# scroll-tech/scroll-prover

Hardware: AMD Instinct MI355X
Metric: BN254 MSM G1-adds/sec at k=26 (higher is better)
Workload: dtype u32 (9x29-bit limbs of 254-bit Montgomery integers; v_mad_u64_u32); 1 GPU; BN254 G1 Pippenger MSM, 2^26 uniform random scalars x synthetic SRS points, inputs resident in HBM; point-range shards over 1 GPU(s), RCCL all-gather of 96-B partials; log_n=26, window_bits=22, windows=12, parallelism=point-range x1, one rank per GPU, srs_window_tables=True

## Files before the change

### scroll-prover_amd/csrc/lib_msm.hip

```cpp
#define ZK_FRSCAN_DEVICE_ONLY 1
#include "msm.hpp"
#define ZK_G2_DEVICE_ONLY 1
#include "msm_g2.hpp"
#include "msm_seg.hpp"
#include "lib_common.hpp"

namespace mi355 {
using mi355zk::Fixup; using mi355zk::PassPlan; using mi355zk::PlanIn; using mi355zk::TableShape;

static_assert(sizeof(fe_t) == 32 && sizeof(g1_affine_t) == 64 && sizeof(g1_jac_t) == 96, "ABI element sizes");
static_assert(sizeof(g1_xyzz_t) == 128 && sizeof(g1_xyzz29_t) == 144, "device record sizes (workspace layout, 16-byte vector accesses)");
static_assert(sizeof(g1_xyzz29_t) == mi355zk::GROUP_G1.rec_bytes && sizeof(g2_xyzz_t) == mi355zk::GROUP_G2.rec_bytes, "the planner's record sizes");

int msm_tu_init_device() {
  HIPCHK(hipFuncSetAttribute((const void *)k_sort_l1_scatter_split<24>, hipFuncAttributeMaxDynamicSharedMemorySize, 160 * 1024));
  HIPCHK(hipFuncSetAttribute((const void *)k_sort_l1_scatter_split<16>, hipFuncAttributeMaxDynamicSharedMemorySize, 160 * 1024));
  HIPCHK(hipFuncSetAttribute((const void *)k_sort_l1_scatter_split<8>, hipFuncAttributeMaxDynamicSharedMemorySize, 160 * 1024));
  HIPCHK(hipFuncSetAttribute((const void *)k_sort_l2_scatter_split<16>, hipFuncAttributeMaxDynamicSharedMemorySize, 160 * 1024));
  HIPCHK(hipFuncSetAttribute((const void *)k_sort_l2_scatter_split<8>, hipFuncAttributeMaxDynamicSharedMemorySize, 160 * 1024));
  return MI355_OK;
}

static PlanIn plan_in() {
  PlanIn in; in.k = static_cast<const mi355zk::Knobs &>(g); in.auto_max_c = g_proc.msm_auto_max_c; in.chunk_min_log = g.msm_chunk_min_log;
// ... 2 lines not shown
}

struct PreTable { const g1_affine_t *table = nullptr; uint64_t row_stride = 0; int c = 0, w = 0; };
static TableShape tab_of(const PreTable *pre) { return pre && pre->table ? TableShape{pre->c, pre->w} : TableShape{}; }
const PreTable *pre_advance(const PreTable *pre, uint64_t lo, PreTable &store) {
  if (!pre) return nullptr;
  store = *pre; if (store.table) store.table += lo;
  return &store;
}

struct Roles {
  const char *prefix; std::string sfx;
  template <class T> int get(const char *name, size_t bytes, T *&ptr) const { return ws_get((std::string(prefix) + name + sfx).c_str(), bytes, (void **)&ptr); }
};

struct MsmStreams { hipStream_t a, b, c; };
struct SpanNames { const char *total, *digits, *sort, *l1, *hist, *l2, *accumulate, *fixup, *tail; };

template <class H> struct PassArgs {
  const typename H::base_t *bases; uint64_t row_stride;
  PolyPtrs inl; const fe_t *const *polys_dev;
  typename H::Ops::out_t *out;
  MsmSlot *slot; MsmStreams st;
  uint32_t set_index = 0, set_count = 1;
  bool skip_tail = false;
  bool normalise = true;
};

struct G1Pass {
  using Ops = G1Ops; using base_t = g1_affine_t;
  static constexpr mi355zk::MsmGroup GROUP = mi355zk::GROUP_G1;
  static constexpr bool FOLD = true, G1_SCHEDULES = true;
  static constexpr SpanNames SPAN{"msm_total", "msm_digits", "msm_sort", "sort_l1", "sort_hist", "sort_l2", "msm_accumulate", "msm_reduce", nullptr};
  static constexpr const char *TRACE = "msm_g1", *N_LIMIT = "msm: n must be < 2^31"; static constexpr double TRACE_BYTES = 96.0;
  static void accumulate(const PassPlan &pl, const PassArgs<G1Pass> &a, const uint32_t *sorted, const uint32_t *offsets, g1_xyzz29_t *buckets, g1_xyzz29_t *part, int32_t *part_id, hipStream_t s) {
    hipLaunchKernelGGL(k_msm_accumulate, dim3(pl.blocks), dim3(256), 0, s, a.bases, sorted, offsets, (uint32_t)pl.nbuckets, buckets, part, part_id, pl.seg_arg, log2_ceil(pl.n), a.row_stride);
  }
};
struct G2Pass {
  using Ops = G2Ops; using base_t = g2_affine_t;
  static constexpr mi355zk::MsmGroup GROUP = mi355zk::GROUP_G2;
  static constexpr bool FOLD = false, G1_SCHEDULES = false;
  static constexpr SpanNames SPAN{"msm_g2_total", "msm_g2_digits", "msm_g2_sort", "g2_sort_l1", "g2_sort_hist", "g2_sort_l2", "msm_g2_accumulate", "msm_g2_fixup", "msm_g2_reduce"};
  static constexpr const char *TRACE = "msm_g2", *N_LIMIT = "msm_g2: n must be < 2^31"; static constexpr double TRACE_BYTES = 160.0;
  static void accumulate(const PassPlan &pl, const PassArgs<G2Pass> &a, const uint32_t *sorted, const uint32_t *offsets, g2_xyzz_t *buckets, g2_xyzz_t *part, int32_t *part_id, hipStream_t s) {
    hipLaunchKernelGGL(k_msm_g2_accumulate, dim3(pl.blocks), dim3(256), 0, s, a.bases, sorted, offsets, (uint32_t)pl.nbuckets, buckets, part, part_id, pl.seg_arg);
  }
};

static void g1_bases(PassArgs<G1Pass> &a, const PassPlan &pl, const g1_affine_t *bases, const PreTable *pre) {
  if (pl.shared) { a.bases = pre->table; a.row_stride = pre->row_stride; } else { a.bases = bases; a.row_stride = 0; }
}

int msm_stage_polys(const fe_t *const *polys_host, uint32_t M, const Roles &ws, hipStream_t s, PolyPtrs &inl, const fe_t **&polys_dev) {
  if (M <= 8) { for (uint32_t m = 0; m < M; m++) inl.p[m] = polys_host[m]; return MI355_OK; }
  CHK(ws.get("polys", (size_t)M * sizeof(void *), polys_dev));
  g.polys_stage.assign(polys_host, polys_host + M);
  HIPCHK(hipMemcpyAsync(polys_dev, g.polys_stage.data(), (size_t)M * sizeof(void *), hipMemcpyHostToDevice, s));
  HIPCHK(hipStreamSynchronize(s));
  return MI355_OK;
}

template <class G, class F> void with_lanes(bool quad, F &&launch) {
  if constexpr (G::QUAD) { if (quad) { launch(std::integral_constant<int, 4>{}); return; } }
  launch(std::integral_constant<int, 1>{});
}

template <class H> int msm_sort_stage(const PassPlan &pl, const MsmPlan &P, const PolyPtrs &inl, const fe_t *const *polys_dev, uint32_t *offsets, uint32_t *sorted, hipStream_t s) {
  const uint64_t emax = pl.emax;
  const uint32_t nbuckets = (uint32_t)pl.nbuckets, M = pl.M;
  SortPlan S; S.n = P.n; S.windows = M * P.windows; S.wpp = P.windows; S.nb = P.nb;
  S.fb = pl.fb; S.cb_bits = pl.cb_bits;
  S.shared = pl.shared ? 1 : 0; S.nshift = log2_ceil(pl.n);
  S.regions = pl.regions; S.t1 = pl.t1; S.t2 = pl.t2;
  const uint32_t tiles1 = pl.tiles1, l2_tiles_max = pl.l2_tiles_max;
  const uint32_t vwindows = M * P.windows;

  uint32_t *enc, *hist, *cursor, *scan_sums, *coarse_hist, *coarse_off, *coarse_cursor, *tile_start;
  CHK(ws_get("msm.digits", emax * 4, (void **)&enc));
  uint32_t *pairs_lo = nullptr; uint16_t *pairs_hi = nullptr;
  CHK(ws_get("msm.pairs_lo", emax * 4 + 64, (void **)&pairs_lo)); CHK(ws_get("msm.pairs_hi", emax * 2 + 64, (void **)&pairs_hi));
  CHK(ws_get("msm.hist", ((size_t)nbuckets + 1) * 4, (void **)&hist));
  CHK(ws_get("msm.cursor", ((size_t)nbuckets + 1) * 4, (void **)&cursor));
  CHK(ws_get("msm.coarse_hist", ((size_t)S.regions + 1) * 4, (void **)&coarse_hist));
  CHK(ws_get("msm.coarse_off", ((size_t)S.regions + 1) * 4, (void **)&coarse_off));
  CHK(ws_get("msm.coarse_cursor", ((size_t)S.regions + 1) * 4, (void **)&coarse_cursor));
  CHK(ws_get("msm.tile_start", ((size_t)S.regions + 1) * 4, (void **)&tile_start));
  const uint32_t scan_n = nbuckets + 1, scan_blocks = ceil_div(scan_n, SCAN_BLOCK * SCAN_ITEMS);
  const uint32_t cscan_n = S.regions + 1, cscan_blocks = ceil_div(cscan_n, SCAN_BLOCK * SCAN_ITEMS);
  CHK(ws_get("msm.scan_sums", (size_t)(scan_blocks + cscan_blocks) * 4, (void **)&scan_sums));
  const int grid_stream = g.prop.multiProcessorCount * 8;
  {
    Scope sc(H::SPAN.digits, s);
    HIPCHK(hipMemsetAsync(coarse_hist, 0, ((size_t)S.regions + 1) * 4, s));
    const dim3 dgrid(grid_stream / M > 0 ? grid_stream / M : 1, M);
    hipLaunchKernelGGL(k_msm_digits<H::FOLD>, dgrid, dim3(256), (size_t)S.regions * 4, s, inl, polys_dev, enc, P, coarse_hist, S.fb, S.cb_bits, S.shared);
  }
  {
    Scope sc(H::SPAN.sort, s);
    HIPCHK(hipMemsetAsync(hist, 0, ((size_t)nbuckets + 1) * 4, s));
    hipLaunchKernelGGL(k_scan_partial, dim3(cscan_blocks), dim3(SCAN_BLOCK), 0, s, coarse_hist, scan_sums + scan_blocks, cscan_n);
    hipLaunchKernelGGL(k_scan_block_sums, dim3(1), dim3(SCAN_BLOCK), 0, s, scan_sums + scan_blocks, cscan_blocks);
    hipLaunchKernelGGL(k_scan_final, dim3(cscan_blocks), dim3(SCAN_BLOCK), 0, s, coarse_hist, scan_sums + scan_blocks, coarse_off, coarse_cursor, cscan_n);
    {
      Scope s1(H::SPAN.l1, s);
      const uint32_t CBp = ((1u << S.cb_bits) + 1) & ~1u;
      const size_t lds1 = (size_t)(3 * CBp + 32 + SORT_SPLIT_TMAX) * 4 + (size_t)S.t1 * 6;
      if (S.t1 == 24576) hipLaunchKernelGGL(k_sort_l1_scatter_split<24>, dim3(tiles1 * vwindows), dim3(1024), lds1, s, enc, coarse_cursor, pairs_lo, pairs_hi, S);
      else if (S.t1 == 16384) hipLaunchKernelGGL(k_sort_l1_scatter_split<16>, dim3(tiles1 * vwindows), dim3(1024), lds1, s, enc, coarse_cursor, pairs_lo, pairs_hi, S);
      else hipLaunchKernelGGL(k_sort_l1_scatter_split<8>, dim3(tiles1 * vwindows), dim3(1024), lds1, s, enc, coarse_cursor, pairs_lo, pairs_hi, S);
    }
    hipLaunchKernelGGL(k_sort_tile_prefix, dim3(1), dim3(SCAN_BLOCK), 0, s, coarse_off, tile_start, S);
    { Scope s2(H::SPAN.hist, s);
    hipLaunchKernelGGL(k_sort_l2_hist_split, dim3(l2_tiles_max), dim3(256), 0, s, (const uint16_t *)pairs_hi, coarse_off, tile_start, hist, S); }
    hipLaunchKernelGGL(k_scan_partial, dim3(scan_blocks), dim3(SCAN_BLOCK), 0, s, hist, scan_sums, scan_n);
    hipLaunchKernelGGL(k_scan_block_sums, dim3(1), dim3(SCAN_BLOCK), 0, s, scan_sums, scan_blocks);
    hipLaunchKernelGGL(k_scan_final, dim3(scan_blocks), dim3(SCAN_BLOCK), 0, s, hist, scan_sums, offsets, cursor, scan_n);
    {
      Scope s3(H::SPAN.l2, s);
      const size_t lds2 = (size_t)(3 * (1u << S.fb) + 32) * 4 + (size_t)S.t2 * 6;
      if (S.t2 == 8192) hipLaunchKernelGGL(k_sort_l2_scatter_split<8>, dim3(l2_tiles_max), dim3(1024), lds2, s, (const uint32_t *)pairs_lo, (const uint16_t *)pairs_hi, coarse_off, tile_start, cursor, sorted, S);
      else hipLaunchKernelGGL(k_sort_l2_scatter_split<16>, dim3(l2_tiles_max), dim3(1024), lds2, s, (const uint32_t *)pairs_lo, (const uint16_t *)pairs_hi, coarse_off, tile_start, cursor, sorted, S);
    }
  }
  return MI355_OK;
}

template <class G> int msm_segfix_levels(const int32_t *part_id, const typename G::rec_t *part, uint32_t tn, typename G::rec_t *buckets, hipStream_t s, const Roles &ws) {
  using rec_t = typename G::rec_t;
  uint32_t N = 2 * tn; const uint32_t waves1 = ceil_div(N, 64);
  const size_t cap = (size_t)2 * waves1 + (size_t)waves1 / 8 + 512;
  int32_t *lv_ids; rec_t *lv_recs;
  CHK(ws.get("segfix_ids", cap * 4, lv_ids)); CHK(ws.get("segfix_recs", cap * sizeof(rec_t), lv_recs));
  const int32_t *cur_ids = part_id; const rec_t *cur_recs = part; size_t used = 0;
  while (N > 64) {
    const uint32_t waves = ceil_div(N, 64);
    hipLaunchKernelGGL(k_msm_segfix<G>, dim3(ceil_div(N, 256)), dim3(256), 0, s, cur_ids, cur_recs, N, buckets, lv_ids + used, lv_recs + used, 0);
    cur_ids = lv_ids + used; cur_recs = lv_recs + used; used += (size_t)2 * waves; N = 2 * waves;
  }
  hipLaunchKernelGGL(k_msm_segfix<G>, dim3(1), dim3(64), 0, s, cur_ids, cur_recs, N, buckets, (int32_t *)nullptr, (rec_t *)nullptr, 1);
  return MI355_OK;
}

struct FixupLists {
  uint32_t *big_list, *big_count, *huge_list, *huge_count; g1_xyzz29_t *huge_part;
  int get(const PassPlan &pl, const Roles &ws) {
    CHK(ws.get("big_list", ((size_t)pl.big_cap * 3 + 1) * 4, big_list)); big_count = big_list + (size_t)pl.big_cap * 3;
    CHK(ws.get("huge_list", ((size_t)pl.huge_cap * 3 + 1) * 4, huge_list)); huge_count = huge_list + (size_t)pl.huge_cap * 3;
    return ws.get("huge_part", (size_t)pl.huge_cap * FIXUP_SLICES * sizeof(g1_xyzz29_t), huge_part);
  }
};
static void msm_fixup_per_bucket(const PassPlan &pl, const FixupLists &fl, const uint32_t *offsets, g1_xyzz29_t *buckets, g1_xyzz29_t *part, int32_t *part_id, hipStream_t s) {
  const uint32_t nbuckets = (uint32_t)pl.nbuckets;
  auto fixup = [&](auto kernel, uint64_t threads) {
    hipLaunchKernelGGL(kernel, dim3(ceil_div(threads, 256)), dim3(256), 0, s, offsets, nbuckets, buckets, part, part_id, pl.seg_arg, pl.tn, fl.big_list, fl.big_count, pl.big_cap, fl.huge_list, fl.huge_count, pl.huge_cap, pl.serial_max, pl.huge_min);
  };
  if (pl.fixup == Fixup::Quad) fixup(k_msm_fixup<4, 4>, (uint64_t)nbuckets * 16);
  else if (pl.fixup == Fixup::FourLanes) fixup(k_msm_fixup<4, 1>, (uint64_t)nbuckets * 4);
  else fixup(k_msm_fixup<1, 1>, nbuckets);
  hipLaunchKernelGGL(k_msm_fixup_big, dim3(pl.big_cap), dim3(256), 0, s, buckets, part, part_id, fl.big_list, fl.big_count);
  hipLaunchKernelGGL(k_msm_fixup_huge, dim3(pl.huge_cap * FIXUP_SLICES), dim3(256), 0, s, part, part_id, fl.huge_list, fl.huge_count, fl.huge_part, pl.huge_cap);
  hipLaunchKernelGGL(k_msm_fixup_huge_fold, dim3(pl.huge_cap), dim3(64), 0, s, buckets, fl.huge_list, fl.huge_count, (const g1_xyzz29_t *)fl.huge_part);
}

template <class G> int msm_reduce_tail(const PassPlan &pl, const typename G::rec_t *buckets, typename G::out_t *out_dev, bool normalise, hipStream_t s, const Roles &ws) {
  using rec_t = typename G::rec_t;
  const uint32_t nb = 1u << (pl.c - 1), wpp = pl.wpp(), sets = pl.sets(), chunks_per_set = pl.chunks_per_set, nchunks = chunks_per_set * sets;
  rec_t *chunk_out, *tree_a, *tree_b, *window_sums;
  CHK(ws.get("chunk_out", (size_t)nchunks * sizeof(rec_t), chunk_out));
  { const size_t lvl = (size_t)ceil_div(chunks_per_set, 64 * TREE_PER_THREAD) * sets + 1;
    CHK(ws.get("tree_a", lvl * sizeof(rec_t), tree_a)); CHK(ws.get("tree_b", lvl * sizeof(rec_t), tree_b)); }
  CHK(ws.get("window_sums", (size_t)sets * sizeof(rec_t), window_sums));
  with_lanes<G>(pl.quad_sums, [&](auto q) {
    constexpr int Q = decltype(q)::value;
    hipLaunchKernelGGL((k_msm_bucket_reduce<G, Q>), dim3(ceil_div((uint64_t)nchunks * Q, 128)), dim3(128), 0, s, buckets, chunk_out, nb, sets, pl.chunk);
  });
  const rec_t *cur = chunk_out; uint32_t cnt = chunks_per_set; rec_t *bufs[2] = {tree_a, tree_b}; int which = 0;
  while (true) {
    const bool coop = G::QUAD && pl.tree_quad(cnt);
    const uint32_t outn = ceil_div(cnt, (coop ? 64u : 256u) * TREE_PER_THREAD);
    rec_t *dst = outn == 1 ? window_sums : bufs[which];
    with_lanes<G>(coop, [&](auto q) { hipLaunchKernelGGL((k_msm_tree_sum<G, decltype(q)::value>), dim3(outn, sets), dim3(256), 0, s, cur, cnt, dst, outn); });
    if (outn == 1) break;
    cur = dst; cnt = outn; which ^= 1;
  }
  with_lanes<G>(pl.quad_final, [&](auto q) {
    hipLaunchKernelGGL((k_msm_final<G, decltype(q)::value>), dim3(pl.M), dim3(64), 0, s, (const rec_t *)window_sums, wpp, pl.shared ? 0u : pl.c, out_dev, normalise ? 1 : 0);
  });
  HIPCHK(hipGetLastError());
  return MI355_OK;
}

template <class H> int msm_pass(const PassPlan &pl, const PassArgs<H> &a) {
// ... 721 lines not shown
```

### scroll-prover_amd/csrc/msm.hpp

```cpp
#pragma once
#include "fp_asm.hpp"
#include "g1_29.hpp"
#include "frscan.hpp"
#include "msm_plan.hpp"

namespace zk {

#if defined(__HIPCC__)

struct MsmPlan {
  uint32_t n;
  uint32_t c;
  uint32_t windows;
  uint32_t nb;
  uint32_t seg;
  uint32_t batch;
};

__device__ __forceinline__ g1_affine_t load_affine(const g1_affine_t *p) {
  g1_affine_t r; r.x = g_load(&p->x); r.y = g_load(&p->y); return r;
}
__device__ __forceinline__ g1_affine_t load_affine_nt(const g1_affine_t *p) {
  const uint32_t *q = reinterpret_cast<const uint32_t *>(p); g1_affine_t r;
#pragma unroll
  for (int i = 0; i < 8; i++) { r.x.l[i] = __builtin_nontemporal_load(q + i); r.y.l[i] = __builtin_nontemporal_load(q + 8 + i); }
  return r;
}
__device__ __forceinline__ g1_xyzz_t load_xyzz(const g1_xyzz_t *p) {
  g1_xyzz_t r; r.x = g_load(&p->x); r.y = g_load(&p->y); r.zz = g_load(&p->zz); r.zzz = g_load(&p->zzz); return r;
}
__device__ __forceinline__ void store_xyzz(g1_xyzz_t *p, const g1_xyzz_t &v) {
  g_store(&p->x, v.x); g_store(&p->y, v.y); g_store(&p->zz, v.zz); g_store(&p->zzz, v.zzz);
}

__device__ __forceinline__ void store_xyzz29(g1_xyzz29_t *p, const g1_xyzz29_t &v) {
  const uint32_t *w = reinterpret_cast<const uint32_t *>(&v); uint4 *q = reinterpret_cast<uint4 *>(p);
#pragma unroll
  for (int i = 0; i < 9; i++) q[i] = make_uint4(w[4 * i], w[4 * i + 1], w[4 * i + 2], w[4 * i + 3]);
}
__device__ __forceinline__ g1_xyzz29_t load_xyzz29(const g1_xyzz29_t *p) {
  g1_xyzz29_t v; uint32_t *w = reinterpret_cast<uint32_t *>(&v); const uint4 *q = reinterpret_cast<const uint4 *>(p);
#pragma unroll
  for (int i = 0; i < 9; i++) { const uint4 a = q[i]; w[4 * i] = a.x; w[4 * i + 1] = a.y; w[4 * i + 2] = a.z; w[4 * i + 3] = a.w; }
  return v;
}

__device__ __forceinline__ g1_xyzz29_t shfl_down_xyzz29(const g1_xyzz29_t &v, uint32_t o) {
  g1_xyzz29_t r; const uint32_t *s = reinterpret_cast<const uint32_t *>(&v); uint32_t *d = reinterpret_cast<uint32_t *>(&r);
#pragma unroll
  for (int i = 0; i < 36; i++) d[i] = __shfl_down(s[i], o);
  return r;
}
__device__ __forceinline__ g1_xyzz29_t shfl_xor_xyzz29(const g1_xyzz29_t &v, uint32_t o) {
  g1_xyzz29_t r; const uint32_t *s = reinterpret_cast<const uint32_t *>(&v); uint32_t *d = reinterpret_cast<uint32_t *>(&r);
#pragma unroll
  for (int i = 0; i < 36; i++) d[i] = __shfl_xor(s[i], o);
  return r;
}

template <int J> __device__ __forceinline__ fe29_t quad_bcast(const fe29_t &v) {
  fe29_t r;
#pragma unroll
  for (int i = 0; i < 9; i++) {
    int x = __builtin_amdgcn_mov_dpp((int)v.l[i], J * 0x55, 0xf, 0xf, true);
    asm volatile("" : "+v"(x));
    r.l[i] = (uint32_t)x;
  }
  return r;
}
__device__ __forceinline__ fe29_t quad_sel(uint32_t q, const fe29_t a0, const fe29_t a1, const fe29_t a2, const fe29_t a3) {
  fe29_t r;
#pragma unroll
  for (int i = 0; i < 9; i++) { const uint32_t x0 = a0.l[i], x1 = a1.l[i], x2 = a2.l[i], x3 = a3.l[i]; const uint32_t lo = q & 1u ? x1 : x0, hi = q & 1u ? x3 : x2; r.l[i] = q & 2u ? hi : lo; }
  return r;
}
__device__ __forceinline__ g1_xyzz29_t g1_xyzz29_dbl_q4(const g1_xyzz29_t &a) {
  if (g1_xyzz29_is_identity(a)) return a;
  const uint32_t q = threadIdx.x & 3u;
  const fe29_t xt = Fq29::reduce_small(Fq29::normalise(a.x));
  const fe29_t yc = Fq29::carry(a.y);
  const fe29_t U = Fq29::dbl(yc);
  fe29_t m = Fq29::mul_c(quad_sel(q, U, xt, U, xt), quad_sel(q, U, xt, U, xt));
  const fe29_t V = quad_bcast<0>(m), xx = quad_bcast<1>(m);
  const fe29_t M = Fq29::carry(Fq29::add(Fq29::dbl(xx), xx));
  m = Fq29::mul_c(quad_sel(q, U, xt, M, V), quad_sel(q, V, V, M, a.zz));
  const fe29_t W = quad_bcast<0>(m), S = quad_bcast<1>(m), MM = quad_bcast<2>(m), ZZ3 = quad_bcast<3>(m);
  g1_xyzz29_t r;
  r.x = Fq29::sub8(MM, Fq29::dbl(S));
  const fe29_t t = Fq29::sub16(S, r.x);
  m = Fq29::mul_c(quad_sel(q, M, W, W, W), quad_sel(q, t, yc, a.zzz, a.zzz));
  r.y = Fq29::sub4(quad_bcast<0>(m), quad_bcast<1>(m));
  r.zz = ZZ3; r.zzz = quad_bcast<2>(m);
  return r;
}
__device__ __forceinline__ void g1_xyzz29_add_q4(g1_xyzz29_t &acc, const g1_xyzz29_t &o) {
  if (g1_xyzz29_is_identity(o)) return;
  if (g1_xyzz29_is_identity(acc)) { acc = o; return; }
  const uint32_t q = threadIdx.x & 3u;
  fe29_t m = Fq29::mul_c(quad_sel(q, acc.x, acc.y, o.x, o.y), quad_sel(q, o.zz, o.zzz, acc.zz, acc.zzz));
  const fe29_t U1 = quad_bcast<0>(m), S1 = quad_bcast<1>(m), U2 = quad_bcast<2>(m), S2 = quad_bcast<3>(m);
  const fe29_t Pd = Fq29::sub4(U2, U1), Rd = Fq29::sub4(S2, S1);
  m = Fq29::mul_c(quad_sel(q, Pd, Rd, acc.zz, acc.zzz), quad_sel(q, Pd, Rd, o.zz, o.zzz));
  const fe29_t PP = quad_bcast<0>(m), RR = quad_bcast<1>(m), ZZ12 = quad_bcast<2>(m), ZZZ12 = quad_bcast<3>(m);
  const fe29_t one = Fq29::one();
  m = Fq29::mul_c(quad_sel(q, Pd, U1, ZZ12, Rd), quad_sel(q, PP, PP, PP, one));
  const fe29_t PPP = quad_bcast<0>(m), Q = quad_bcast<1>(m), ZZ3 = quad_bcast<2>(m), Rone = quad_bcast<3>(m);
  if (Fq29::is_zero_tight(ZZ3)) {
    if (Fq29::is_zero_tight(Rone)) acc = g1_xyzz29_dbl_q4(acc);
    else acc = g1_xyzz29_identity();
    return;
  }
  const fe29_t X3 = Fq29::sub4_8(RR, PPP, Fq29::dbl(Q));
  const fe29_t t = Fq29::sub16(Q, X3);
  m = Fq29::mul_c(quad_sel(q, Rd, S1, ZZZ12, ZZZ12), quad_sel(q, t, PPP, PPP, PPP));
  acc.x = X3; acc.y = Fq29::sub4(quad_bcast<0>(m), quad_bcast<1>(m));
  acc.zz = ZZ3; acc.zzz = quad_bcast<2>(m);
}
template <int Q> __device__ __forceinline__ void g1_vadd(g1_xyzz29_t &acc, const g1_xyzz29_t &o) { if (Q == 4) g1_xyzz29_add_q4(acc, o); else g1_xyzz29_add(acc, o); }
template <int Q> __device__ __forceinline__ g1_xyzz29_t g1_vdbl(const g1_xyzz29_t &a) { return Q == 4 ? g1_xyzz29_dbl_q4(a) : g1_xyzz29_dbl(a); }

__device__ __forceinline__ void msm_emit_result(const g1_xyzz_t &acc, g1_jac_t *out, int normalise) {
  if (normalise) { *out = g1_xyzz_to_jac_normalised(acc); return; }
  g1_jac_t r;
  if (g1_xyzz_is_identity(acc)) { r.x = Fq::zero(); r.y = Fq::zero(); r.z = Fq::zero(); }
  else { r.x = FqPs::mul(acc.x, FqPs::sqr(acc.zz)); r.y = FqPs::mul(acc.y, FqPs::sqr(acc.zzz)); r.z = acc.zzz; }
  *out = r;
}

struct G1Ops {
  using rec_t = g1_xyzz29_t; using out_t = g1_jac_t;
  static constexpr bool QUAD = true;
  static constexpr const char *ROLE = "msm.";
  static __device__ __forceinline__ rec_t identity() { return g1_xyzz29_identity(); }
  static __device__ __forceinline__ rec_t load(const rec_t *p) { return load_xyzz29(p); }
  static __device__ __forceinline__ void store(rec_t *p, const rec_t &v) { store_xyzz29(p, v); }
  template <int Q> static __device__ __forceinline__ void add(rec_t &acc, const rec_t &o) { g1_vadd<Q>(acc, o); }
  template <int Q> static __device__ __forceinline__ rec_t dbl(const rec_t &a) { return g1_vdbl<Q>(a); }
  static __device__ __forceinline__ rec_t shfl_down(const rec_t &v, uint32_t o) { return shfl_down_xyzz29(v, o); }
  static __device__ __forceinline__ void emit(const rec_t &acc, out_t *out, int normalise) { msm_emit_result(g1_xyzz29_to_sat(acc), out, normalise); }
};

struct PolyPtrs { const fe_t *p[8]; };
template <bool FOLD>
__global__ void __launch_bounds__(256) k_msm_digits(PolyPtrs inl, const fe_t *const *__restrict__ polys, uint32_t *__restrict__ enc, MsmPlan P,
                                                     uint32_t *__restrict__ coarse_hist, uint32_t fb, uint32_t cb_bits, uint32_t shared) {
  extern __shared__ uint32_t hist_lds[];
  const uint32_t CB = 1u << cb_bits, per_poly = (shared ? 1u : P.windows) * CB, regions = P.batch * per_poly;
  for (uint32_t b = threadIdx.x; b < regions; b += blockDim.x) hist_lds[b] = 0;
  __syncthreads();
  const uint32_t stride = gridDim.x * blockDim.x, m = blockIdx.y;
  const fe_t *__restrict__ poly = polys ? polys[m] : inl.p[m];
  const uint32_t half = 1u << (P.c - 1), mask = (1u << P.c) - 1;
  for (uint32_t i = blockIdx.x * blockDim.x + threadIdx.x; i < P.n; i += stride) {
    const fe_t k = Fr::redc(g_load(&poly[i]));
    fe_t t; { uint32_t borrow = 0;
#pragma unroll
      for (int q = 0; q < 8; q++) { const uint64_t d = (uint64_t)FrP::mod(q) - k.l[q] - borrow; t.l[q] = (uint32_t)d; borrow = (uint32_t)(d >> 63); } }
    bool flip = false;
#pragma unroll
    for (int q = 7; q >= 0; q--) { if (t.l[q] != k.l[q]) { flip = FOLD && t.l[q] < k.l[q]; break; } }
    const uint32_t sign_flip = flip ? 0x80000000u : 0u;
    uint32_t l0 = flip ? t.l[0] : k.l[0], l1 = flip ? t.l[1] : k.l[1], l2 = flip ? t.l[2] : k.l[2], l3 = flip ? t.l[3] : k.l[3];
    uint32_t l4 = flip ? t.l[4] : k.l[4], l5 = flip ? t.l[5] : k.l[5], l6 = flip ? t.l[6] : k.l[6], l7 = flip ? t.l[7] : k.l[7];
    uint32_t carry = 0;
    for (uint32_t w = 0; w < P.windows; w++) {
      const uint32_t raw = (l0 & mask) + carry;
      l0 = __funnelshift_r(l0, l1, P.c); l1 = __funnelshift_r(l1, l2, P.c); l2 = __funnelshift_r(l2, l3, P.c); l3 = __funnelshift_r(l3, l4, P.c);
      l4 = __funnelshift_r(l4, l5, P.c); l5 = __funnelshift_r(l5, l6, P.c); l6 = __funnelshift_r(l6, l7, P.c); l7 >>= P.c;
      uint32_t e;
      if (raw > half) { e = (1u << P.c) - raw; if (e) e |= 0x80000000u; carry = 1; } else { e = raw; carry = 0; }
      if (e) e ^= sign_flip;
      enc[((uint64_t)m * P.windows + w) * P.n + i] = e;
      if (e) atomicAdd(&hist_lds[m * per_poly + (shared ? 0 : w * CB) + (((e & 0x7fffffffu) - 1) >> fb)], 1u);
    }
  }
  __syncthreads();
  for (uint32_t b = threadIdx.x; b < regions; b += blockDim.x) if (hist_lds[b]) atomicAdd(&coarse_hist[b], hist_lds[b]);
}

__device__ __forceinline__ uint32_t block_exclusive_scan(uint32_t v, uint32_t *lds, uint32_t &total) {
  const uint32_t lane = threadIdx.x & 63, wave = threadIdx.x >> 6;
  uint32_t x = v;
  for (uint32_t o = 1; o < 64; o <<= 1) { uint32_t y = __shfl_up(x, o); if (lane >= o) x += y; }
  if (lane == 63) lds[wave] = x;
  __syncthreads();
  if (wave == 0) { uint32_t s = lane < (blockDim.x >> 6) ? lds[lane] : 0; for (uint32_t o = 1; o < 16; o <<= 1) { uint32_t y = __shfl_up(s, o); if (lane >= o) s += y; } if (lane < 16) lds[16 + lane] = s; }
  __syncthreads();
  const uint32_t wave_off = wave ? lds[16 + wave - 1] : 0;
  total = lds[16 + (blockDim.x >> 6) - 1];
  __syncthreads();
  return wave_off + x - v;
}
__global__ void __launch_bounds__(SCAN_BLOCK) k_scan_partial(const uint32_t *__restrict__ in, uint32_t *__restrict__ block_sums, uint32_t n) {
  __shared__ uint32_t lds[32];
  const uint32_t base = blockIdx.x * SCAN_BLOCK * SCAN_ITEMS + threadIdx.x * SCAN_ITEMS;
  uint32_t s = 0;
  for (uint32_t k = 0; k < SCAN_ITEMS; k++) if (base + k < n) s += in[base + k];
  uint32_t total; block_exclusive_scan(s, lds, total);
  if (threadIdx.x == 0) block_sums[blockIdx.x] = total;
}
__global__ void __launch_bounds__(SCAN_BLOCK) k_scan_block_sums(uint32_t *block_sums, uint32_t nblocks) {
  __shared__ uint32_t lds[32];
  __shared__ uint32_t running;
  if (threadIdx.x == 0) running = 0;
  __syncthreads();
  for (uint32_t base = 0; base < nblocks; base += SCAN_BLOCK) {
    const uint32_t i = base + threadIdx.x;
    const uint32_t v = i < nblocks ? block_sums[i] : 0;
    uint32_t total; const uint32_t ex = block_exclusive_scan(v, lds, total);
    const uint32_t r = running;
    if (i < nblocks) block_sums[i] = r + ex;
    __syncthreads();
    if (threadIdx.x == 0) running = r + total;
    __syncthreads();
  }
}
__global__ void __launch_bounds__(SCAN_BLOCK) k_scan_final(const uint32_t *__restrict__ in, const uint32_t *__restrict__ block_sums, uint32_t *__restrict__ out_a, uint32_t *__restrict__ out_b, uint32_t n) {
  __shared__ uint32_t lds[32];
  const uint32_t base = blockIdx.x * SCAN_BLOCK * SCAN_ITEMS + threadIdx.x * SCAN_ITEMS;
  uint32_t v[SCAN_ITEMS], s = 0;
  for (uint32_t k = 0; k < SCAN_ITEMS; k++) { v[k] = base + k < n ? in[base + k] : 0; s += v[k]; }
  uint32_t total; uint32_t ex = block_exclusive_scan(s, lds, total) + block_sums[blockIdx.x];
  for (uint32_t k = 0; k < SCAN_ITEMS; k++) if (base + k < n) { out_a[base + k] = ex; out_b[base + k] = ex; ex += v[k]; }
}

struct SortPlan { uint32_t n, windows , wpp , nb, fb, cb_bits, t1, t2, regions, shared, nshift ; };

__device__ __forceinline__ uint32_t tile_bin_offsets(const uint32_t *h, uint32_t *lstart, uint32_t (&gb)[4], uint32_t nbins, uint32_t *global_cursor, uint32_t *scratch32) {
  const uint32_t bpt = (nbins + 1023) >> 10, b0 = threadIdx.x * bpt;
  uint32_t local[4], sum = 0;
  for (uint32_t k = 0; k < 4; k++) { local[k] = (k < bpt && b0 + k < nbins) ? h[b0 + k] : 0; sum += local[k]; }
  uint32_t total; uint32_t ex = block_exclusive_scan(sum, scratch32, total);
  for (uint32_t k = 0; k < 4; k++) { gb[k] = 0; if (k < bpt && b0 + k < nbins) { lstart[b0 + k] = ex; if (local[k]) gb[k] = atomicAdd(&global_cursor[b0 + k], local[k]); ex += local[k]; } }
  return total;
}
__device__ __forceinline__ void tile_bin_publish(uint32_t *gbase, const uint32_t *lstart, const uint32_t (&gb)[4], uint32_t nbins) {
  const uint32_t bpt = (nbins + 1023) >> 10, b0 = threadIdx.x * bpt;
  for (uint32_t k = 0; k < 4; k++) if (k < bpt && b0 + k < nbins) gbase[b0 + k] = gb[k] - lstart[b0 + k];
}
template <int EPT> __global__ void __launch_bounds__(1024) k_sort_l1_scatter_split(const uint32_t *__restrict__ enc, uint32_t *__restrict__ coarse_cursor, uint32_t *__restrict__ pairs_lo,
                                                                                    uint16_t *__restrict__ pairs_hi, SortPlan S) {
  extern __shared__ uint32_t sm[];
  const uint32_t CB = 1u << S.cb_bits, CBp = (CB + 1) & ~1u, fmask = (1u << S.fb) - 1;
  const uint32_t spare = 16u - S.fb, rmask = (1u << spare) - 1, tcount = (CB + rmask) >> spare;
  uint32_t *h = sm, *lstart = sm + CBp, *gbase = sm + 2 * CBp, *scratch32 = sm + 3 * CBp, *T = sm + 3 * CBp + 32;
  uint32_t *stage_lo = T + SORT_SPLIT_TMAX;
  uint16_t *stage_hi = reinterpret_cast<uint16_t *>(stage_lo + 1024 * EPT);
  const uint32_t tiles1 = (S.n + S.t1 - 1) / S.t1;
  const uint32_t w = blockIdx.x / tiles1, j = blockIdx.x - w * tiles1;
  for (uint32_t b = threadIdx.x; b < CB; b += 1024) h[b] = 0;
  __syncthreads();
  const uint32_t i0 = j * S.t1, i1 = min(S.n, i0 + S.t1);
  const uint32_t *plane = enc + (uint64_t)w * S.n;
  uint32_t e[EPT], rank[EPT];
#pragma unroll
  for (int k = 0; k < EPT; k++) {
    const uint32_t i = i0 + k * 1024 + threadIdx.x;
    e[k] = i < i1 ? plane[i] : 0;
  }
  asm volatile("s_waitcnt vmcnt(0)" ::: "memory");
#pragma unroll
  for (int k = 0; k < EPT; k++) if (e[k]) rank[k] = atomicAdd(&h[((e[k] & 0x7fffffffu) - 1) >> S.fb], 1u);
  __syncthreads();
  const uint32_t m_poly = w / S.wpp, w_in = w - m_poly * S.wpp;
  uint32_t gb[4];
  const uint32_t total = tile_bin_offsets(h, lstart, gb, CB, coarse_cursor + (S.shared ? m_poly * CB : w * CB), scratch32);
  const uint32_t idx_base = S.shared ? w_in << S.nshift : 0;
  __syncthreads();
  for (uint32_t k = threadIdx.x; k < tcount; k += 1024) T[k] = lstart[k << spare];
#pragma unroll
  for (int k = 0; k < EPT; k++) if (e[k]) {
    const uint32_t bucket = (e[k] & 0x7fffffffu) - 1, i = i0 + k * 1024 + threadIdx.x, bin = bucket >> S.fb, pos = lstart[bin] + rank[k];
    stage_lo[pos] = (idx_base + i) | (e[k] & 0x80000000u);
    stage_hi[pos] = (uint16_t)((bucket & fmask) | ((bin & rmask) << S.fb));
  }
  tile_bin_publish(gbase, lstart, gb, CB);
  __syncthreads();
  uint32_t k = 0;
  for (uint32_t sidx = threadIdx.x; sidx < total; sidx += 1024) {
    const uint32_t key = stage_hi[sidx];
    while (k + 1 < tcount && T[k + 1] <= sidx) k++;
    const uint32_t bin = (k << spare) | (key >> S.fb), pos = gbase[bin] + sidx;
    pairs_lo[pos] = stage_lo[sidx]; pairs_hi[pos] = (uint16_t)(key & fmask);
  }
}
__global__ void __launch_bounds__(SCAN_BLOCK) k_sort_tile_prefix(const uint32_t *__restrict__ coarse_off, uint32_t *__restrict__ tile_start, SortPlan S) {
  __shared__ uint32_t lds[32];
  __shared__ uint32_t running;
  if (threadIdx.x == 0) running = 0;
  __syncthreads();
  for (uint32_t base = 0; base < S.regions; base += SCAN_BLOCK) {
    const uint32_t r = base + threadIdx.x;
    const uint32_t v = r < S.regions ? (coarse_off[r + 1] - coarse_off[r] + S.t2 - 1) / S.t2 : 0;
    uint32_t total; const uint32_t ex = block_exclusive_scan(v, lds, total);
    const uint32_t run = running;
    if (r < S.regions) tile_start[r] = run + ex;
    __syncthreads();
    if (threadIdx.x == 0) running = run + total;
    __syncthreads();
  }
  if (threadIdx.x == 0) tile_start[S.regions] = running;
}
__device__ __forceinline__ bool sort_l2_tile(const uint32_t *__restrict__ coarse_off, const uint32_t *__restrict__ tile_start, const SortPlan &S, uint32_t &region, uint32_t &s, uint32_t &e) {
  const uint32_t total = tile_start[S.regions], per_xcd = (total + 7) >> 3, q = blockIdx.x >> 3;
  const uint32_t tile = (blockIdx.x & 7) * per_xcd + q;
  if (q >= per_xcd || tile >= total) return false;
  uint32_t lo = 0, hi = S.regions;
  while (hi - lo > 1) { const uint32_t mid = (lo + hi) >> 1; if (tile_start[mid] <= tile) lo = mid; else hi = mid; }
  region = lo;
  s = coarse_off[lo] + (tile - tile_start[lo]) * S.t2;
  e = min(coarse_off[lo + 1], s + S.t2);
  return true;
}
__global__ void __launch_bounds__(256) k_sort_l2_hist_split(const uint16_t *__restrict__ pairs_hi, const uint32_t *__restrict__ coarse_off, const uint32_t *__restrict__ tile_start,
                                                            uint32_t *__restrict__ hist, SortPlan S) {
  __shared__ uint32_t h[SORT_MAX_BINS];
  uint32_t region, s, e;
  if (!sort_l2_tile(coarse_off, tile_start, S, region, s, e)) return;
  const uint32_t FB = 1u << S.fb;
  for (uint32_t b = threadIdx.x; b < FB; b += blockDim.x) h[b] = 0;
  __syncthreads();
  const uint32_t a0 = min(e, (s + 7u) & ~7u), a1 = a0 + ((e - a0) & ~7u);
  for (uint32_t p = s + threadIdx.x; p < a0; p += blockDim.x) atomicAdd(&h[pairs_hi[p]], 1u);
  for (uint32_t q = a0 + 8u * threadIdx.x; q < a1; q += 8u * blockDim.x) {
    const uint4 v = *reinterpret_cast<const uint4 *>(pairs_hi + q);
    atomicAdd(&h[v.x & 0xffffu], 1u); atomicAdd(&h[v.x >> 16], 1u); atomicAdd(&h[v.y & 0xffffu], 1u); atomicAdd(&h[v.y >> 16], 1u);
    atomicAdd(&h[v.z & 0xffffu], 1u); atomicAdd(&h[v.z >> 16], 1u); atomicAdd(&h[v.w & 0xffffu], 1u); atomicAdd(&h[v.w >> 16], 1u);
  }
  for (uint32_t p = a1 + threadIdx.x; p < e; p += blockDim.x) atomicAdd(&h[pairs_hi[p]], 1u);
  __syncthreads();
  for (uint32_t b = threadIdx.x; b < FB; b += blockDim.x) if (h[b]) atomicAdd(&hist[(region << S.fb) + b], h[b]);
}
template <int EPT> __global__ void __launch_bounds__(1024) k_sort_l2_scatter_split(const uint32_t *__restrict__ pairs_lo, const uint16_t *__restrict__ pairs_hi, const uint32_t *__restrict__ coarse_off,
                                                                                    const uint32_t *__restrict__ tile_start, uint32_t *__restrict__ cursor, uint32_t *__restrict__ sorted, SortPlan S) {
  extern __shared__ uint32_t sm[];
  const uint32_t FB = 1u << S.fb;
  uint32_t *h = sm, *lstart = sm + FB, *gbase = sm + 2 * FB, *scratch32 = sm + 3 * FB, *stage = sm + 3 * FB + 32;
  uint32_t region, s, e;
  if (!sort_l2_tile(coarse_off, tile_start, S, region, s, e)) return;
  for (uint32_t b = threadIdx.x; b < FB; b += 1024) h[b] = 0;
  __syncthreads();
  uint32_t idx[EPT], fine[EPT], rank[EPT];
#pragma unroll
  for (int k = 0; k < EPT; k++) {
    const uint32_t p = s + k * 1024 + threadIdx.x;
    fine[k] = 0xffffffffu;
    if (p < e) { idx[k] = pairs_lo[p]; fine[k] = pairs_hi[p]; }
  }
  asm volatile("s_waitcnt vmcnt(0)" ::: "memory");
#pragma unroll
  for (int k = 0; k < EPT; k++) if (fine[k] != 0xffffffffu) rank[k] = atomicAdd(&h[fine[k]], 1u);
  __syncthreads();
  uint32_t gb[4];
  const uint32_t total = tile_bin_offsets(h, lstart, gb, FB, cursor + (region << S.fb), scratch32);
  __syncthreads();
  uint16_t *stage_bin = reinterpret_cast<uint16_t *>(stage + 1024 * EPT);
#pragma unroll
  for (int k = 0; k < EPT; k++) if (fine[k] != 0xffffffffu) { const uint32_t pos = lstart[fine[k]] + rank[k]; stage[pos] = idx[k]; stage_bin[pos] = (uint16_t)fine[k]; }
  tile_bin_publish(gbase, lstart, gb, FB);
  __syncthreads();
  for (uint32_t sidx = threadIdx.x; sidx < total; sidx += 1024) {
    const uint32_t b = stage_bin[sidx];
    sorted[gbase[b] + sidx] = stage[sidx];
  }
}

__device__ __forceinline__ uint32_t msm_seg_eff(uint32_t total, uint32_t threads, uint32_t seg_arg) {
  const uint32_t seg_max = seg_arg & 0x1fffu, seg_min = (seg_arg >> 13) & 0x1fffu, fill_pct = (seg_arg >> 26) * 2;
  const uint64_t target = ((uint64_t)threads * (fill_pct > 100u ? 100u : fill_pct) + 99) / 100;
  uint32_t sg = (uint32_t)(((uint64_t)total + target - 1) / (target ? target : 1));
  sg = sg < seg_min ? seg_min : sg;
  return sg > seg_max ? seg_max : sg;
}
template <class G, class B> __device__ __forceinline__ void msm_segment_walk(const B &bases, const uint32_t *__restrict__ sorted, const uint32_t *__restrict__ offsets, uint32_t nbuckets,
                                                                              typename G::rec_t *__restrict__ bucket_sums, typename G::rec_t *__restrict__ part, int32_t *__restrict__ part_id, uint32_t seg_arg,
                                                                              uint32_t t, uint32_t threads) {
  const uint32_t total = offsets[nbuckets];
  const uint32_t seg = msm_seg_eff(total, threads, seg_arg);
  const uint64_t start64 = (uint64_t)t * seg;
  if (start64 >= total) { part_id[2 * t] = -1; part_id[2 * t + 1] = -1; return; }
  const uint32_t start = (uint32_t)start64, end = (uint32_t)min((uint64_t)total, start64 + seg);
  uint32_t lo = 0, hi = nbuckets;
  while (hi - lo > 1) { const uint32_t mid = (lo + hi) >> 1; if (offsets[mid] <= start) lo = mid; else hi = mid; }
  uint32_t b = lo, b_start = offsets[b], b_end = offsets[b + 1];
  int32_t id_first = -1, id_last = -1;
  typename G::rec_t acc = G::identity();
  uint32_t ent = sorted[start];
  uint32_t ent_next = start + 1 < end ? sorted[start + 1] : 0;
  typename B::base_t p = bases.load(ent);
  for (uint32_t pos = start; pos < end; pos++) {
    typename B::base_t p_next = p;
    if (pos + 1 < end) { ent_next = sorted[pos + 1]; p_next = bases.load(ent_next); }
    if (pos >= b_end) {
      if (b_start >= start) G::store(&bucket_sums[b], acc);
      else { G::store(&part[2 * (uint64_t)t], acc); id_first = (int32_t)b; }
      acc = G::identity();
      b++; b_start = b_end; b_end = offsets[b + 1];
      if (pos >= b_end) {
        uint32_t l2 = b, h2 = nbuckets;
        while (h2 - l2 > 1) { const uint32_t mid = (l2 + h2) >> 1; if (offsets[mid] <= pos) l2 = mid; else h2 = mid; }
        b = l2; b_start = offsets[b]; b_end = offsets[b + 1];
      }
    }
    bases.madd(acc, p, (ent >> 31) != 0);
    ent = ent_next; p = p_next;
  }
  if (b_start >= start && b_end <= end) G::store(&bucket_sums[b], acc);
  else if (b_start < start) { G::store(&part[2 * (uint64_t)t], acc); id_first = (int32_t)b; }
  else { G::store(&part[2 * (uint64_t)t + 1], acc); id_last = (int32_t)b; }
  part_id[2 * t] = id_first; part_id[2 * t + 1] = id_last;
}
struct G1Bases {
  using base_t = g1_affine_t;
  const g1_affine_t *__restrict__ bases; uint32_t nshift; uint64_t row_stride;
  __device__ __forceinline__ const g1_affine_t *base_of(uint32_t e) const {
    const uint32_t gi = e & 0x7fffffffu;
    if (row_stride == 0) return &bases[gi];
    const uint32_t w = gi >> nshift;
    return &bases[(uint64_t)w * row_stride + (gi & ((1u << nshift) - 1))];
  }
  __device__ __forceinline__ g1_affine_t load(uint32_t e) const { return load_affine(base_of(e)); }
  __device__ __forceinline__ void madd(g1_xyzz29_t &acc, const g1_affine_t &p, bool neg) const { g1_xyzz29_madd(acc, p, neg); }
};
struct G1AccOps : G1Ops {
  static __device__ __forceinline__ void store(rec_t *p, rec_t v) { g1_xyzz29_negx_to_plain(v); store_xyzz29(p, v); }
};
__global__ void __launch_bounds__(256) k_msm_accumulate(const g1_affine_t *__restrict__ bases, const uint32_t *__restrict__ sorted, const uint32_t *__restrict__ offsets,
                                                        uint32_t nbuckets, g1_xyzz29_t *__restrict__ bucket_sums, g1_xyzz29_t *__restrict__ part, int32_t *__restrict__ part_id, uint32_t seg_arg,
                                                        uint32_t nshift, uint64_t row_stride) {
  msm_segment_walk<G1AccOps>(G1Bases{bases, nshift, row_stride}, sorted, offsets, nbuckets, bucket_sums, part, part_id, seg_arg, blockIdx.x * blockDim.x + threadIdx.x, gridDim.x * blockDim.x);
}

constexpr uint32_t FIXUP_SERIAL_MAX = 32;
template <int Q = 1> __device__ __forceinline__ void fixup_take29(g1_xyzz29_t &acc, const g1_xyzz29_t *__restrict__ part, const int32_t *__restrict__ part_id, uint32_t t, uint32_t b) {
  if (part_id[2 * t] == (int32_t)b) g1_vadd<Q>(acc, load_xyzz29(&part[2 * (uint64_t)t]));
  else if (part_id[2 * t + 1] == (int32_t)b) g1_vadd<Q>(acc, load_xyzz29(&part[2 * (uint64_t)t + 1]));
}
// ... 261 lines not shown
```

Measured before the change: 12.64 billion G1-adds/s.

## Split coarse sort cursors into per-XCD groups to cut global atomic contention

Partitions L1 sort tiles and digit-histogram counting into 8 interleaved groups (matching blockIdx%8 XCD placement), each with its own coarse histogram and cursor slot. Blocks on the same XCD then bump cursors that other XCDs never touch, so cross-die atomic traffic on shared cache lines should drop. The coarse scan grows by the group factor and the digit kernel iterates a remapped point index with padded spans, which adds some index arithmetic and skipped iterations.

```diff
diff --git a/scroll-prover_amd/csrc/lib_msm.hip b/scroll-prover_amd/csrc/lib_msm.hip
--- a/scroll-prover_amd/csrc/lib_msm.hip
+++ b/scroll-prover_amd/csrc/lib_msm.hip
@@ -108,19 +108,20 @@
   CHK(ws_get("msm.pairs_lo", emax * 4 + 64, (void **)&pairs_lo)); CHK(ws_get("msm.pairs_hi", emax * 2 + 64, (void **)&pairs_hi));
   CHK(ws_get("msm.hist", ((size_t)nbuckets + 1) * 4, (void **)&hist));
   CHK(ws_get("msm.cursor", ((size_t)nbuckets + 1) * 4, (void **)&cursor));
-  CHK(ws_get("msm.coarse_hist", ((size_t)S.regions + 1) * 4, (void **)&coarse_hist));
-  CHK(ws_get("msm.coarse_off", ((size_t)S.regions + 1) * 4, (void **)&coarse_off));
-  CHK(ws_get("msm.coarse_cursor", ((size_t)S.regions + 1) * 4, (void **)&coarse_cursor));
+  const uint32_t cscan_n = S.regions * SORT_GROUPS + 1;
+  CHK(ws_get("msm.coarse_hist", (size_t)cscan_n * 4, (void **)&coarse_hist));
+  CHK(ws_get("msm.coarse_off", (size_t)cscan_n * 4, (void **)&coarse_off));
+  CHK(ws_get("msm.coarse_cursor", (size_t)cscan_n * 4, (void **)&coarse_cursor));
   CHK(ws_get("msm.tile_start", ((size_t)S.regions + 1) * 4, (void **)&tile_start));
   const uint32_t scan_n = nbuckets + 1, scan_blocks = ceil_div(scan_n, SCAN_BLOCK * SCAN_ITEMS);
-  const uint32_t cscan_n = S.regions + 1, cscan_blocks = ceil_div(cscan_n, SCAN_BLOCK * SCAN_ITEMS);
+  const uint32_t cscan_blocks = ceil_div(cscan_n, SCAN_BLOCK * SCAN_ITEMS);
   CHK(ws_get("msm.scan_sums", (size_t)(scan_blocks + cscan_blocks) * 4, (void **)&scan_sums));
   const int grid_stream = g.prop.multiProcessorCount * 8;
   {
     Scope sc(H::SPAN.digits, s);
-    HIPCHK(hipMemsetAsync(coarse_hist, 0, ((size_t)S.regions + 1) * 4, s));
-    const dim3 dgrid(grid_stream / M > 0 ? grid_stream / M : 1, M);
-    hipLaunchKernelGGL(k_msm_digits<H::FOLD>, dgrid, dim3(256), (size_t)S.regions * 4, s, inl, polys_dev, enc, P, coarse_hist, S.fb, S.cb_bits, S.shared);
+    HIPCHK(hipMemsetAsync(coarse_hist, 0, (size_t)cscan_n * 4, s));
+    const dim3 dgrid(std::max<uint32_t>(grid_stream / M / SORT_GROUPS, 1) * SORT_GROUPS, M);
+    hipLaunchKernelGGL(k_msm_digits<H::FOLD>, dgrid, dim3(256), (size_t)S.regions * 4, s, inl, polys_dev, enc, P, coarse_hist, S.fb, S.cb_bits, S.shared, S.t1);
   }
   {
     Scope sc(H::SPAN.sort, s);
@@ -132,9 +133,9 @@
       Scope s1(H::SPAN.l1, s);
       const uint32_t CBp = ((1u << S.cb_bits) + 1) & ~1u;
       const size_t lds1 = (size_t)(3 * CBp + 32 + SORT_SPLIT_TMAX) * 4 + (size_t)S.t1 * 6;
-      if (S.t1 == 24576) hipLaunchKernelGGL(k_sort_l1_scatter_split<24>, dim3(tiles1 * vwindows), dim3(1024), lds1, s, enc, coarse_cursor, pairs_lo, pairs_hi, S);
-      else if (S.t1 == 16384) hipLaunchKernelGGL(k_sort_l1_scatter_split<16>, dim3(tiles1 * vwindows), dim3(1024), lds1, s, enc, coarse_cursor, pairs_lo, pairs_hi, S);
-      else hipLaunchKernelGGL(k_sort_l1_scatter_split<8>, dim3(tiles1 * vwindows), dim3(1024), lds1, s, enc, coarse_cursor, pairs_lo, pairs_hi, S);
+      if (S.t1 == 24576) hipLaunchKernelGGL(k_sort_l1_scatter_split<24>, dim3(sort_l1_grid(tiles1, vwindows)), dim3(1024), lds1, s, enc, coarse_cursor, pairs_lo, pairs_hi, S);
+      else if (S.t1 == 16384) hipLaunchKernelGGL(k_sort_l1_scatter_split<16>, dim3(sort_l1_grid(tiles1, vwindows)), dim3(1024), lds1, s, enc, coarse_cursor, pairs_lo, pairs_hi, S);
+      else hipLaunchKernelGGL(k_sort_l1_scatter_split<8>, dim3(sort_l1_grid(tiles1, vwindows)), dim3(1024), lds1, s, enc, coarse_cursor, pairs_lo, pairs_hi, S);
     }
     hipLaunchKernelGGL(k_sort_tile_prefix, dim3(1), dim3(SCAN_BLOCK), 0, s, coarse_off, tile_start, S);
     { Scope s2(H::SPAN.hist, s);
diff --git a/scroll-prover_amd/csrc/msm.hpp b/scroll-prover_amd/csrc/msm.hpp
--- a/scroll-prover_amd/csrc/msm.hpp
+++ b/scroll-prover_amd/csrc/msm.hpp
@@ -2,6 +2,7 @@
 #include "fp_asm.hpp"
 #include "g1_29.hpp"
 #include "frscan.hpp"
+#include "sort_groups.hpp"
 #include "msm_plan.hpp"
 
 namespace zk {
@@ -143,15 +144,18 @@
 struct PolyPtrs { const fe_t *p[8]; };
 template <bool FOLD>
 __global__ void __launch_bounds__(256) k_msm_digits(PolyPtrs inl, const fe_t *const *__restrict__ polys, uint32_t *__restrict__ enc, MsmPlan P,
-                                                     uint32_t *__restrict__ coarse_hist, uint32_t fb, uint32_t cb_bits, uint32_t shared) {
+                                                     uint32_t *__restrict__ coarse_hist, uint32_t fb, uint32_t cb_bits, uint32_t shared, uint32_t t1) {
   extern __shared__ uint32_t hist_lds[];
   const uint32_t CB = 1u << cb_bits, per_poly = (shared ? 1u : P.windows) * CB, regions = P.batch * per_poly;
   for (uint32_t b = threadIdx.x; b < regions; b += blockDim.x) hist_lds[b] = 0;
   __syncthreads();
-  const uint32_t stride = gridDim.x * blockDim.x, m = blockIdx.y;
+  const uint32_t grp = blockIdx.x % SORT_GROUPS, stride = gridDim.x / SORT_GROUPS * blockDim.x, m = blockIdx.y;
+  const uint32_t span = sort_group_span((P.n + t1 - 1) / t1, t1);
   const fe_t *__restrict__ poly = polys ? polys[m] : inl.p[m];
   const uint32_t half = 1u << (P.c - 1), mask = (1u << P.c) - 1;
-  for (uint32_t i = blockIdx.x * blockDim.x + threadIdx.x; i < P.n; i += stride) {
+  for (uint32_t f = blockIdx.x / SORT_GROUPS * blockDim.x + threadIdx.x; f < span; f += stride) {
+    const uint32_t i = sort_group_point(f, grp, t1);
+    if (i >= P.n) continue;
     const fe_t k = Fr::redc(g_load(&poly[i]));
     fe_t t; { uint32_t borrow = 0;
 #pragma unroll
@@ -175,7 +179,7 @@
     }
   }
   __syncthreads();
-  for (uint32_t b = threadIdx.x; b < regions; b += blockDim.x) if (hist_lds[b]) atomicAdd(&coarse_hist[b], hist_lds[b]);
+  for (uint32_t b = threadIdx.x; b < regions; b += blockDim.x) if (hist_lds[b]) atomicAdd(&coarse_hist[b * SORT_GROUPS + grp], hist_lds[b]);
 }
 
 __device__ __forceinline__ uint32_t block_exclusive_scan(uint32_t v, uint32_t *lds, uint32_t &total) {
@@ -226,12 +230,12 @@
 
 struct SortPlan { uint32_t n, windows , wpp , nb, fb, cb_bits, t1, t2, regions, shared, nshift ; };
 
-__device__ __forceinline__ uint32_t tile_bin_offsets(const uint32_t *h, uint32_t *lstart, uint32_t (&gb)[4], uint32_t nbins, uint32_t *global_cursor, uint32_t *scratch32) {
+__device__ __forceinline__ uint32_t tile_bin_offsets(const uint32_t *h, uint32_t *lstart, uint32_t (&gb)[4], uint32_t nbins, uint32_t *global_cursor, uint32_t cursor_stride, uint32_t *scratch32) {
   const uint32_t bpt = (nbins + 1023) >> 10, b0 = threadIdx.x * bpt;
   uint32_t local[4], sum = 0;
   for (uint32_t k = 0; k < 4; k++) { local[k] = (k < bpt && b0 + k < nbins) ? h[b0 + k] : 0; sum += local[k]; }
   uint32_t total; uint32_t ex = block_exclusive_scan(sum, scratch32, total);
-  for (uint32_t k = 0; k < 4; k++) { gb[k] = 0; if (k < bpt && b0 + k < nbins) { lstart[b0 + k] = ex; if (local[k]) gb[k] = atomicAdd(&global_cursor[b0 + k], local[k]); ex += local[k]; } }
+  for (uint32_t k = 0; k < 4; k++) { gb[k] = 0; if (k < bpt && b0 + k < nbins) { lstart[b0 + k] = ex; if (local[k]) gb[k] = atomicAdd(&global_cursor[(b0 + k) * cursor_stride], local[k]); ex += local[k]; } }
   return total;
 }
 __device__ __forceinline__ void tile_bin_publish(uint32_t *gbase, const uint32_t *lstart, const uint32_t (&gb)[4], uint32_t nbins) {
@@ -246,8 +250,9 @@
   uint32_t *h = sm, *lstart = sm + CBp, *gbase = sm + 2 * CBp, *scratch32 = sm + 3 * CBp, *T = sm + 3 * CBp + 32;
   uint32_t *stage_lo = T + SORT_SPLIT_TMAX;
   uint16_t *stage_hi = reinterpret_cast<uint16_t *>(stage_lo + 1024 * EPT);
-  const uint32_t tiles1 = (S.n + S.t1 - 1) / S.t1;
-  const uint32_t w = blockIdx.x / tiles1, j = blockIdx.x - w * tiles1;
+  const SortL1Block blk = sort_l1_block(blockIdx.x, (S.n + S.t1 - 1) / S.t1);
+  const uint32_t w = blk.w, j = blk.j;
+  if ((uint64_t)j * S.t1 >= S.n) return;
   for (uint32_t b = threadIdx.x; b < CB; b += 1024) h[b] = 0;
   __syncthreads();
   const uint32_t i0 = j * S.t1, i1 = min(S.n, i0 + S.t1);
@@ -264,7 +269,7 @@
   __syncthreads();
   const uint32_t m_poly = w / S.wpp, w_in = w - m_poly * S.wpp;
   uint32_t gb[4];
-  const uint32_t total = tile_bin_offsets(h, lstart, gb, CB, coarse_cursor + (S.shared ? m_poly * CB : w * CB), scratch32);
+  const uint32_t total = tile_bin_offsets(h, lstart, gb, CB, coarse_cursor + (S.shared ? m_poly * CB : w * CB) * SORT_GROUPS + j % SORT_GROUPS, SORT_GROUPS, scratch32);
   const uint32_t idx_base = S.shared ? w_in << S.nshift : 0;
   __syncthreads();
   for (uint32_t k = threadIdx.x; k < tcount; k += 1024) T[k] = lstart[k << spare];
@@ -291,7 +296,7 @@
   __syncthreads();
   for (uint32_t base = 0; base < S.regions; base += SCAN_BLOCK) {
     const uint32_t r = base + threadIdx.x;
-    const uint32_t v = r < S.regions ? (coarse_off[r + 1] - coarse_off[r] + S.t2 - 1) / S.t2 : 0;
+    const uint32_t v = r < S.regions ? (coarse_off[(r + 1) * SORT_GROUPS] - coarse_off[r * SORT_GROUPS] + S.t2 - 1) / S.t2 : 0;
     uint32_t total; const uint32_t ex = block_exclusive_scan(v, lds, total);
     const uint32_t run = running;
     if (r < S.regions) tile_start[r] = run + ex;
@@ -308,8 +313,8 @@
   uint32_t lo = 0, hi = S.regions;
   while (hi - lo > 1) { const uint32_t mid = (lo + hi) >> 1; if (tile_start[mid] <= tile) lo = mid; else hi = mid; }
   region = lo;
-  s = coarse_off[lo] + (tile - tile_start[lo]) * S.t2;
-  e = min(coarse_off[lo + 1], s + S.t2);
+  s = coarse_off[lo * SORT_GROUPS] + (tile - tile_start[lo]) * S.t2;
+  e = min(coarse_off[(lo + 1) * SORT_GROUPS], s + S.t2);
   return true;
 }
 __global__ void __launch_bounds__(256) k_sort_l2_hist_split(const uint16_t *__restrict__ pairs_hi, const uint32_t *__restrict__ coarse_off, const uint32_t *__restrict__ tile_start,
@@ -352,7 +357,7 @@
   for (int k = 0; k < EPT; k++) if (fine[k] != 0xffffffffu) rank[k] = atomicAdd(&h[fine[k]], 1u);
   __syncthreads();
   uint32_t gb[4];
-  const uint32_t total = tile_bin_offsets(h, lstart, gb, FB, cursor + (region << S.fb), scratch32);
+  const uint32_t total = tile_bin_offsets(h, lstart, gb, FB, cursor + (region << S.fb), 1, scratch32);
   __syncthreads();
   uint16_t *stage_bin = reinterpret_cast<uint16_t *>(stage + 1024 * EPT);
 #pragma unroll
diff --git a/scroll-prover_amd/csrc/sort_groups.hpp b/scroll-prover_amd/csrc/sort_groups.hpp
--- /dev/null
+++ b/scroll-prover_amd/csrc/sort_groups.hpp
@@ -0,0 +1,27 @@
+#pragma once
+#include <cstdint>
+
+#if defined(__HIPCC__)
+#define ZK_SORT_HD __host__ __device__ __forceinline__
+#else
+#define ZK_SORT_HD inline
+#endif
+
+namespace zk {
+constexpr uint32_t SORT_GROUPS = 8;
+
+struct SortL1Block { uint32_t w, j; };
+ZK_SORT_HD uint32_t sort_l1_tiles_per_group(uint32_t tiles1) { return (tiles1 + SORT_GROUPS - 1) / SORT_GROUPS; }
+ZK_SORT_HD uint32_t sort_l1_grid(uint32_t tiles1, uint32_t vwindows) { return SORT_GROUPS * sort_l1_tiles_per_group(tiles1) * vwindows; }
+ZK_SORT_HD SortL1Block sort_l1_block(uint32_t b, uint32_t tiles1) {
+  const uint32_t x = b % SORT_GROUPS, q = b / SORT_GROUPS, tpg = sort_l1_tiles_per_group(tiles1);
+  SortL1Block r; r.w = q / tpg; r.j = SORT_GROUPS * (q % tpg) + x;
+  return r;
+}
+
+ZK_SORT_HD uint32_t sort_group_span(uint32_t tiles1, uint32_t t1) { return sort_l1_tiles_per_group(tiles1) * t1; }
+ZK_SORT_HD uint32_t sort_group_point(uint32_t f, uint32_t g, uint32_t t1) {
+  const uint32_t jj = f / t1, off = f - jj * t1;
+  return (SORT_GROUPS * jj + g) * t1 + off;
+}
+}
```

Measured after the change: 12.66 billion G1-adds/s (median of 5 runs). Within noise of the previous version (+0.1%).
